# mtumalan/VisionTransformer

Measured on AMD Instinct MI355X. Metric: images/sec (512×512) ViT-B/16 seg, 1/2/4/8 MI355X + mask argmax match, higher is better.
Workload: dtype f32

## Files before the change

visiontransformer_amd/csrc/common.hpp:

```cpp
#pragma once
#include <hip/hip_runtime.h>
#include <stdint.h>

#include "../../include/vitseg.h"

namespace vitseg {

constexpr int WAVE = 64;

typedef float f32x4 __attribute__((ext_vector_type(4)));
typedef float f32x16 __attribute__((ext_vector_type(16)));
typedef short bf16x8 __attribute__((ext_vector_type(8)));
typedef short bf16x4 __attribute__((ext_vector_type(4)));

void set_error(const char* fmt, ...);
int hip_fail(hipError_t e, const char* what);

enum Opt {
    OPT_NO_F32P = 0,
    OPT_NO_P8,
    OPT_NO_H16P,
    OPT_NO_RAGGED_P8,
    OPT_NO_DROPMASK,
    OPT_DROPW_LIMIT_MB,
    OPT_UPSAMPLE_GLOBAL,
    OPT_BF16_TILES,
    OPT_F32P_NOINL,
    OPT_GN,
    OPT_NO_MASK2,
    OPT_NO_SMALL,
    OPT_SMALL_VARIANT,
    OPT_SMALL_MAX_ROWS,
    OPT_CONV_DMA,
    OPT_COUNT
};
long opt(int id);

#define VITSEG_CHECK_ARG(cond, code, ...) \
    do {                                  \
        if (!(cond)) {                    \
            ::vitseg::set_error(__VA_ARGS__); \
            return (code);                \
        }                                 \
    } while (0)

#define VITSEG_LAUNCH_CHECK(what)                               \
    do {                                                        \
        hipError_t e__ = hipGetLastError();                     \
        if (e__ != hipSuccess) return ::vitseg::hip_fail(e__, what); \
    } while (0)

inline size_t up256(size_t v) { return (v + 255) & ~(size_t)255; }

__device__ __forceinline__ int xcd_remap(int bid, int nwg) {
    const int q = nwg >> 3, r = nwg & 7, xcd = bid & 7, idx = bid >> 3;
    const int base = (xcd < r) ? xcd * (q + 1) : r * (q + 1) + (xcd - r) * q;
    return base + idx;
}

struct AttnTile {
    int rt, head, b;
};
__device__ __forceinline__ AttnTile attn_tile(int ntiles, int A) {
    const int t = xcd_remap(blockIdx.x, gridDim.x);
    const int bh = t / ntiles;
    AttnTile r;
    r.rt = t - bh * ntiles;
    r.b = bh / A;
    r.head = bh - r.b * A;
    return r;
}

__host__ __device__ __forceinline__ unsigned fmix32(unsigned h) {
    h ^= h >> 16;
    h *= 0x85ebca6bu;
    h ^= h >> 13;
    h *= 0xc2b2ae35u;
    h ^= h >> 16;
    return h;
}
__host__ __device__ __forceinline__ unsigned drop_key(unsigned seed, unsigned stream, unsigned major) {
    return fmix32(seed ^ (stream * 0x9E3779B1u) ^ (major * 0x85EBCA77u));
}
__host__ __device__ __forceinline__ unsigned mad24(unsigned a, unsigned k, unsigned c) {
#if defined(__HIP_DEVICE_COMPILE__)
    return __umul24(a, k) + c;
// ... 209 lines not shown
```

visiontransformer_amd/csrc/forward.hip:

```cpp
#include "kernels.hpp"
#include "profile.hpp"
#include "forward.hpp"

namespace vitseg {

using namespace plan;

long small_max_rows() {
    const long v = opt(OPT_SMALL_MAX_ROWS);
    return v > 0 ? v : SMALL_MAX_ROWS;
}

bool small_applies(const vitseg_config* cfg, int batch, int precision) {
    Shape s;
    if (precision == VITSEG_F32X3 || opt(OPT_NO_SMALL) || check_config(cfg, &s)) return false;
    const long rows = (long)batch * s.N;
    if (!(rows < small_max_rows() && s.D % 64 == 0 && s.I % 32 == 0 && s.I > s.D && s.S % 4 == 0)) return false;
    const long lim16 = opt(OPT_SMALL_MAX_ROWS) > 0 ? opt(OPT_SMALL_MAX_ROWS) : small_max_rows_16(s.N);
    if (precision != VITSEG_F32 && !(s.I % 64 == 0 && attn_small_infer(s.Np) && rows < lim16)) return false;
    if (precision != VITSEG_F32 && ((s.D / small_splits(s.D, s.D)) % 64 || (s.I / small_splits(s.D, s.I)) % 64)) return false;
    return true;
}

namespace {
// ... 22 lines not shown
    }
    if (int rc = launch_cls_rows(wt(f, VITSEG_T_CLS), f.pos, X, f.batch, s.Np, s.D, f.st)) return rc;
    if (f.drop_p > 0.f) return launch_dropout_rows(X, X, 0, Mp + f.batch, s.D, drop(f, 0, 0), f.st);
    return VITSEG_OK;
}

int head_conv_gemm(const Fwd& f) {
    const Shape& s = f.s;
    const int Mp = f.batch * s.Np, D = s.D;
    GemmArgs g{};
    g.A = f.hf; g.W = wg(f, VITSEG_T_HEAD0_W); g.bias = wt(f, VITSEG_T_HEAD0_B); g.C = f.F;
    g.M = Mp; g.N = MID; g.K = 9 * D; g.lda = 0; g.ldc = MID;
    g.g = s.g; g.Np = s.Np; g.D = D;
    g.zeros = f.zeros;
    if (f.h16) {
        hipError_t e = hipMemsetAsync((void*)f.zeros, 0, 256, f.st);
        if (e != hipSuccess) return hip_fail(e, "hipMemsetAsync(zero page)");
    }
    ProfScope ps(f.prof.conv3, 2.0 * g.M * g.N * g.K, f.st);
    if (f.conv_dma && !f.h16 && !f.x3 && D % 32 == 0 && opt(OPT_CONV_DMA) && (size_t)(Mp + 128) * D * 4 < 0x7fffffffull) {
        SGemm c{};
        c.A = (const float*)f.hf; c.W = wt(f, VITSEG_T_HEAD0_W); c.bias = wt(f, VITSEG_T_HEAD0_B); c.C = f.F;
        c.M = Mp; c.N = MID; c.K = D; c.lda = D; c.ldw = 9 * D; c.ldc = MID; c.splits = 1;
        c.g = s.g; c.Np = s.Np;
        return launch_gemm_f32s(c, SE_RELU, SA_CONV3_ALL, f.st);
    }
    return f.h16 ? launch_gemm_bf16(g, A_CONV3, EPI_RELU, f.st, f.h16 == 2) : launch_gemm_f32(g, A_CONV3, EPI_RELU, f.st, f.x3);
}

int head_1x1(const Fwd& f) {
    const Shape& s = f.s;
    const size_t Mp = (size_t)f.batch * s.Np;
    ProfScope ps(f.prof.head1x1, (double)Mp * MID * 4 + (double)f.batch * s.C * s.Np * 4, f.st);
    return launch_head1x1(f.F, wt(f, VITSEG_T_HEAD2_W), wt(f, VITSEG_T_HEAD2_B), f.Z, f.batch, s.Np, s.C, f.st);
}

int upsample(const Fwd& f) {
    const Shape& s = f.s;
    if (!f.logits && !f.mask) return VITSEG_OK;
    const double px = (double)f.batch * s.S * s.S;
    ProfScope ps(f.prof.upsample, (f.logits ? px * s.C * 4 : 0.0) + (f.mask ? px : 0.0) + (double)f.batch * s.C * s.Np * 4, f.st);
    return launch_upsample(f.Z, f.logits, f.mask, f.batch, s.C, s.g, s.S, f.st);
}

}

int walk_large(const Fwd& f) {
    const Shape& s = f.s;
    const int Mp = f.batch * s.Np, Mt = Mp + f.batch, D = s.D, I = s.I;
    hipStream_t st = f.st;
    int rc;
    if ((rc = embed_gemm(f, f.layer(0).xin, f.h16 ? 1 : f.x3))) return rc;
    const int thin_rows = f.thin_rows ? thin_cls_rows(Mp, f.batch) : 0;
    auto gemm = [&](const void* A, int w, int b, int l, const float* R, void* C, int N, int K, int epi, int kind,
                    DropArgs dr = DropArgs{}, void* aux = nullptr) {
        GemmArgs g{};
        g.A = A; g.W = wg(f, w, l); g.bias = wt(f, b, l); g.R = R; g.C = C; g.aux = aux; g.drop = dr;
        g.M = Mt; g.N = N; g.K = K; g.lda = K; g.ldc = N;
        if (f.whole_split || thin_rows) {
            g.thin_rows = thin_rows;
            g.thin_scratch = f.scratch;
            g.thin_capacity = f.scratch_floats;
        }
        ProfScope ps(kind, 2.0 * g.M * g.N * g.K, st);
        if (f.fc1_train && epi == EPI_GELU) return launch_gemm_bf16_train(g, EPI_GELU, st);
        return f.h16 ? launch_gemm_bf16(g, A_PLAIN, epi, st, f.h16 == 2) : launch_gemm_f32(g, A_PLAIN, epi, st, f.x3);
    };
    auto lnorm = [&](const float* X, int w, int b, int l, void* H, int rows) {
        ProfScope ps(f.prof.ln, (double)rows * D * (f.h16 ? 6 : 8), st);
        return launch_layernorm(X, wt(f, w, l), wt(f, b, l), H, rows, D, f.eps, f.h16, st);
    };
    const bool mlp1 = f.prof.mlp_one_scope;
    for (int l = 0; l < s.L; ++l) {
        const LayerIO io = f.layer(l);
        if ((rc = lnorm(io.xin, VITSEG_T_LN1_W, VITSEG_T_LN1_B, l, io.h1, Mt))) return rc;
        if ((rc = gemm(io.h1, VITSEG_T_WQKV, VITSEG_T_BQKV, l, nullptr, io.qkv, 3 * D, D, EPI_BIAS, f.prof.qkv))) return rc;
        {
            ProfScope ps(f.prof.attn, 4.0 * f.batch * s.A * (double)s.N * s.N * 64, st);
            const DropArgs dr = drop(f, l, 1);
            if (io.dropw && (rc = launch_attn_dropmask((unsigned*)io.dropw, f.batch, s.Np, s.A, dr, st))) return rc;
            rc = f.h16 ? launch_attention_bf16(io.qkv, io.ctx, io.lse, f.batch, s.Np, s.A, dr, st, f.h16 == 2, io.dropw)
                       : launch_attention_f32((const float*)io.qkv, (float*)io.ctx, io.lse, f.batch, s.Np, s.A, dr, st, f.x3 != 0);
            if (rc) return rc;
        }
        if ((rc = gemm(io.ctx, VITSEG_T_WO, VITSEG_T_BO, l, io.xin, io.xmid, D, D, EPI_RESADD, f.prof.oproj, drop(f, l, 2))))
            return rc;
        if ((rc = lnorm(io.xmid, VITSEG_T_LN2_W, VITSEG_T_LN2_B, l, io.h2, Mt))) return rc;
        ProfScope ps(mlp1 ? f.prof.fc1 : -1, 4.0 * Mt * D * I, st);
        if ((rc = gemm(io.h2, VITSEG_T_W1, VITSEG_T_B1, l, nullptr, io.uact, I, D, EPI_GELU, mlp1 ? -1 : f.prof.fc1, DropArgs{},
                       io.upre)))
            return rc;
        if ((rc = gemm(io.uact, VITSEG_T_W2, VITSEG_T_B2, l, io.xmid, io.xout, D, I, EPI_RESADD, mlp1 ? -1 : f.prof.fc2,
                       drop(f, l, 3))))
            return rc;
    }
    if ((rc = lnorm(f.layer(s.L - 1).xout, VITSEG_T_LNF_W, VITSEG_T_LNF_B, 0, f.hf, Mp))) return rc;
    if ((rc = head_conv_gemm(f)) || (rc = head_1x1(f))) return rc;
    return upsample(f);
}

int walk_small(const Fwd& f) {
    const Shape& s = f.s;
    const int Mp = f.batch * s.Np, Mt = Mp + f.batch, D = s.D;
    hipStream_t st = f.st;
    float* part = f.scratch;
    const size_t dstride = (size_t)Mt * D;
    int rc;
    auto linear = [&](const void* A, int K, int w, int b, int l, void* C, int N, int epi, void* aux, int kind) {
        SGemm g{};
        g.A = (const float*)A; g.W = (const float*)wg(f, w, l); g.bias = wt(f, b, l); g.C = (float*)C; g.aux = (float*)aux;
        g.h16 = f.h16;
        g.M = Mt; g.N = N; g.K = K; g.lda = K; g.ldw = K; g.ldc = N;
        g.splits = epi == SE_PARTIAL ? small_splits(N, K) : 1;
        g.split_stride = dstride;
        ProfScope ps(kind, 2.0 * g.M * g.N * g.K, st);
        return launch_gemm_f32s(g, epi, SA_PLAIN, st);
    };
    auto rows = [&](float* X, const float* Xres, int splits, const float* bias, DropArgs dr, int lnw, int lnb, int ln_layer,
                    void* H, int ln_rows, int h_fmt, bool embed) {
        SRows r{};
        r.h_fmt = h_fmt;
        r.X = X; r.Xres = Xres == X ? nullptr : Xres; r.partial = part; r.split_stride = dstride; r.splits = splits;
        r.bias = bias; r.drop = dr;
        r.pos = f.pos; r.cls = wt(f, VITSEG_T_CLS); r.lnw = wt(f, lnw, ln_layer); r.lnb = wt(f, lnb, ln_layer); r.H = (float*)H;
        r.rows = Mt; r.Mp = Mp; r.Np = s.Np; r.D = D; r.ln_rows = ln_rows; r.embed = embed ? 1 : 0;
        r.eps = f.eps;
        ProfScope ps(f.prof.ln, (double)Mt * D * 4 * (2 + splits) + (double)ln_rows * D * 4, st);
        return launch_resln(r, st);
    };
    const LayerIO io0 = f.layer(0);
    if ((s.P == 8 || s.P == 16 || s.P == 32) && s.Kp % 32 == 0) {
        SGemm g{};
        g.A = f.x; g.W = wt(f, VITSEG_T_PATCH_W); g.C = part;
        g.M = Mp; g.N = D; g.K = s.Kp; g.lda = 0; g.ldw = s.Kp; g.ldc = D;
        g.splits = small_splits(D, s.Kp); g.split_stride = dstride;
        g.g = s.g; g.Np = s.Np; g.S = s.S; g.P = s.P; g.Cin = s.Cin;
        {
            ProfScope ps(f.prof.patch, 2.0 * g.M * g.N * g.K, st);
            if ((rc = launch_gemm_f32s(g, SE_PARTIAL, SA_PATCH, st))) return rc;
        }
        if ((rc = rows(io0.xin, nullptr, g.splits, wt(f, VITSEG_T_PATCH_B), drop(f, 0, 0), VITSEG_T_LN1_W, VITSEG_T_LN1_B, 0,
                       io0.h1, Mt, f.h16, true)))
            return rc;
    } else {
        if ((rc = embed_gemm(f, io0.xin, 0))) return rc;
        ProfScope ps(f.prof.ln, (double)Mt * D * 8, st);
        if ((rc = launch_layernorm(io0.xin, wt(f, VITSEG_T_LN1_W), wt(f, VITSEG_T_LN1_B), io0.h1, Mt, D, f.eps, f.h16, st)))
            return rc;
    }
// ... 71 lines not shown
```

visiontransformer_amd/csrc/forward.hpp:

```cpp
#pragma once
#include <functional>

#include "plan.hpp"
#include "small.hpp"

namespace vitseg {

struct LayerIO {
    float* xin;
    void* h1;
    void* qkv;
    void* ctx;
    float* lse;
    float* xmid;
    void* h2;
    void* upre;
    void* uact;
    float* xout;
    const unsigned* dropw;
};

struct FwdProf {
    int patch, ln, qkv, attn, oproj, fc1, fc2, conv3, head1x1, upsample;
    bool mlp_one_scope;
};

struct Fwd {
    plan::Shape s;
    const plan::Layout* lay;
    const float* params;
    const void* params_lp;
    const float* pos;
    const float* x;
    int batch;
    float eps;
    hipStream_t st;
    int h16;
    int x3;
    std::function<LayerIO(int)> layer;
    void* hf;
    float* F;
    float* Z;
    const void* zeros;
    float* scratch;
    size_t scratch_floats;
    float* logits;
    uint8_t* mask;
    float drop_p;
    unsigned drop_seed;
    bool thin_rows;
    bool whole_split;
    bool fc1_train;
    bool (*attn_small)(int Np);
    bool head_one_chain;
    bool conv_dma;
    FwdProf prof;
};

int walk_large(const Fwd& f);
int walk_small(const Fwd& f);

enum SmallRole { SMALL_INFER, SMALL_TRAIN_FWD, SMALL_TRAIN_BWD };
size_t small_slab_floats(const plan::Shape& s, size_t Mt, size_t Mp, SmallRole role);

inline int thin_cls_rows(size_t Mp, int batch) { return Mp % 256 == 0 && batch <= THIN_MAX_ROWS ? batch : 0; }

}
```

visiontransformer_amd/csrc/gemm_dispatch.hip:

```cpp
#include "gemm_tiles.hpp"

namespace vitseg {
namespace {

int whole_split_shape(int M, int N, int K, int kstep) { return K % kstep == 0 ? whole_split(M, N, K, kstep) : 0; }

int thin_slices(int K, int kstep) {
    if (K < 256 || K % kstep != 0) return 0;
    const int sl = K / kstep / 4;
    return sl > THIN_MAX_SPLITS ? THIN_MAX_SPLITS : sl < 1 ? 1 : sl;
}

int whole_split_applies(const GemmArgs& a, int epi, int kstep) {
    const int sp = whole_split_shape(a.M, a.N, a.K, kstep);
    const bool ok = sp && a.thin_scratch && (size_t)sp * a.M * a.N <= a.thin_capacity && !a.drop.thresh &&
                    !a.aux && a.splitk <= 1 && a.ldc % 4 == 0 && (epi == EPI_BIAS || epi == EPI_GELU || epi == EPI_RESADD);
    return ok ? sp : 0;
}

int thin_split_applies(const GemmArgs& a, int epi, int kstep) {
    const bool h16 = kstep == 64;
    const int sl = thin_slices(a.K, kstep);
    const bool ok = sl && a.thin_scratch && a.thin_rows > 0 && a.thin_rows <= THIN_MAX_ROWS && a.M > a.thin_rows &&
                    (size_t)sl * a.thin_rows * a.N <= a.thin_capacity && (a.M - a.thin_rows) % BM == 0 &&
                    (h16 || (!a.drop.thresh && !a.aux)) && a.splitk <= 1 && a.ldc % 4 == 0 &&
                    (epi == EPI_BIAS || epi == EPI_GELU || epi == EPI_RESADD || (h16 && epi == EPI_DGELU));
    return ok ? sl : 0;
}

template <typename F>
int sliced(GemmArgs a, int splits, float* scratch, hipStream_t s, F launch) {
    float* out = (float*)a.C;
    if (splits > 1) {
        a.C = scratch;
        a.splitk = splits;
    }
    a.split_stride = (size_t)a.M * a.N;
    if (int rc = launch(a)) return rc;
    return splits > 1 ? launch_splitk_reduce(scratch, out, (size_t)a.M * a.N / 4, splits, s) : VITSEG_OK;
}

enum H16Kernel { HK_NONE, HK_TILE, HK_LARGE, HK_XL, HK_P8, HK_H16P };

struct H16Route {
    H16Kernel body;
    int body_rows;
    int tail_rows;
    int slices;
    int colsum_rows;
};

}

int launch_gemm_f32(const GemmArgs& a_in, int amode, int epi, hipStream_t s, int x3) {
    if (x3 != 1 && x3 != 2) x3 = 0;
    GemmArgs a = a_in;
    if (amode == A_PLAIN) {
        if (const int sp = whole_split_applies(a_in, epi, 32)) {
            a.thin_rows = a_in.M;
            return launch_thin_rows(GT_F32, x3, a, epi, sp, s);
        }
        if (const int sl = thin_split_applies(a_in, epi, 32)) {
            if (int rc = launch_thin_rows(GT_F32, x3, a_in, epi, sl, s)) return rc;
            a.M = a_in.M - a_in.thin_rows;
        }
    }
    a.thin_scratch = nullptr;
    VITSEG_CHECK_ARG(a.M > 0 && a.N > 0 && a.K > 0 && a.K % 4 == 0, VITSEG_EINVAL, "gemm_f32: bad M/N/K %d %d %d", a.M, a.N, a.K);
    VITSEG_CHECK_ARG(a.N % 4 == 0 && a.ldc % 4 == 0, VITSEG_ESHAPE, "gemm: N=%d and ldc=%d must be multiples of 4", a.N, a.ldc);
    if (amode == A_PLAIN) {
        VITSEG_CHECK_ARG(a.lda % 4 == 0, VITSEG_EINVAL, "gemm_f32: lda %% 4");
        if (!x3 && gemm_f32p_applies(a, epi)) return launch_gemm_f32p(a, epi, s);
    } else if (amode == A_PATCH && epi == EPI_POS) {
        VITSEG_CHECK_ARG(a.P % 4 == 0, VITSEG_ESHAPE, "patch size must be a multiple of 4");
    } else if (amode == A_CONV3 && epi == EPI_RELU) {
        VITSEG_CHECK_ARG(a.D % 4 == 0, VITSEG_ESHAPE, "hidden size must be a multiple of 4");
    }
    static const char* const who[3] = {"gemm_f32", "gemm_f32 (x3)", "gemm_f32 (x3, split W)"};
    return launch_gemm_tile(GT_F32, true, amode, epi, x3, a, s, who[x3]);
}

int launch_gemm_f32_bwd(const GemmArgs& a, int amode, int ta, int tb, int epi, hipStream_t s) {
    VITSEG_CHECK_ARG(a.M > 0 && a.N > 0 && a.K > 0, VITSEG_EINVAL, "gemm_bwd: bad M/N/K %d %d %d", a.M, a.N, a.K);
    VITSEG_CHECK_ARG(a.N % 4 == 0 && a.ldc % 4 == 0 && a.lda % 4 == 0 && a.ldw % 4 == 0, VITSEG_ESHAPE,
                     "gemm_bwd: leading dimensions must be multiples of 4");
    VITSEG_CHECK_ARG(ta || a.K % 4 == 0, VITSEG_ESHAPE, "gemm_bwd: K %% 4");
    VITSEG_CHECK_ARG(!ta || a.M % 4 == 0, VITSEG_ESHAPE, "gemm_bwd: M %% 4 for a T-form A");
    return launch_gemm_tile_bwd(amode, ta, tb, epi, a, s);
}

int launch_wgrad_f32(GemmArgs a, float* scratch, hipStream_t s) {
    const int splits = wgrad_splits(a.M, a.N, a.K, 32);
    VITSEG_CHECK_ARG(splits <= 1 || (a.ldc == a.N && scratch), VITSEG_EINVAL, "wgrad: split-K needs a dense output and scratch");
    return sliced(a, splits, scratch, s, [&](const GemmArgs& g) { return launch_gemm_f32_bwd(g, A_PLAIN, 1, 1, EPI_BIAS, s); });
}

static int route_h16(const GemmArgs& a_in, int amode, int epi, H16Route& r) {
    r = H16Route{HK_NONE, 0, 0, 0, 0};
    const bool want_cs = a_in.colsum_out && a_in.colsum_scratch && epi == EPI_DGELU;
    const auto persistent = [&](const GemmArgs& g) {
        r.body = gemm_h16p_applies(g, epi) ? HK_H16P : HK_P8;
        r.body_rows = g.M;
        r.colsum_rows = want_cs ? g.M : 0;
        return VITSEG_OK;
    };
    GemmArgs a = a_in;
    if (amode == A_PLAIN) {
        if (const int sp = whole_split_applies(a_in, epi, 64)) {
            r.tail_rows = a_in.M;
            r.slices = sp;
            return VITSEG_OK;
        }
        if (a_in.M % 256 != 0 && a_in.M % 256 <= 128 && gemm_p8_applies(a_in, epi) &&
            gemm_p8_rounds(a_in.M, a_in.N) == gemm_p8_rounds(a_in.M - a_in.M % 256, a_in.N) && !opt(OPT_NO_RAGGED_P8))
            return persistent(a_in);
        const int sl = (a_in.M - a_in.thin_rows) % LBM == 0 ? thin_split_applies(a_in, epi, 64) : 0;
        if (sl) {
            r.tail_rows = a_in.thin_rows;
            r.slices = sl;
// ... 20 lines not shown
        r.body = xl ? HK_XL : large ? HK_LARGE : HK_TILE;
        if (epi == EPI_BIAS || epi == EPI_GELU || epi == EPI_DGELU || epi == EPI_RESADD) return VITSEG_OK;
    } else if (amode == A_CONV3 && (epi == EPI_RELU || epi == EPI_BIAS)) {
        VITSEG_CHECK_ARG(a.D % 64 == 0 && a.zeros, VITSEG_ESHAPE, "%s must be a multiple of 64",
                         epi == EPI_RELU ? "hidden size" : "channel count");
        r.body = large ? HK_LARGE : HK_TILE;
        return VITSEG_OK;
    }
    set_error("gemm_bf16: unsupported amode/epilogue %d/%d", amode, epi);
    return VITSEG_EINVAL;
}

int launch_gemm_bf16(const GemmArgs& a_in, int amode, int epi, hipStream_t s, bool f16) {
    H16Route r;
    if (int rc = route_h16(a_in, amode, epi, r)) return rc;
    const GemmType type = f16 ? GT_F16 : GT_BF16;
    const bool out_f32 = epi == EPI_RESADD || amode == A_CONV3;
    GemmArgs a = a_in;
    if (r.slices) {
        a.thin_rows = r.tail_rows;
        if (int rc = launch_thin_rows(type, 0, a, epi, r.slices, s)) return rc;
    }
    a.M = r.body_rows;
    a.thin_scratch = nullptr;
    if (!r.colsum_rows) a.colsum_scratch = nullptr;
    int rc = VITSEG_OK;
    switch (r.body) {
        case HK_NONE: break;
        case HK_P8: rc = launch_gemm_p8(a, epi, s, f16); break;
        case HK_H16P: rc = launch_gemm_h16p(a, s, f16); break;
        case HK_XL: rc = launch_gemm_large(f16, amode, epi, 256, a, s, "gemm_bf16"); break;
        case HK_LARGE: rc = launch_gemm_large(f16, amode, epi, 128, a, s, "gemm_bf16"); break;
        case HK_TILE: rc = launch_gemm_tile(type, out_f32, amode, epi, 0, a, s, "gemm_bf16");
    }
    if (rc) return rc;
    if (r.tail_rows && !r.slices) {
        GemmArgs t = a;
        const auto row = [&](const void* p, size_t esz) { return (char*)p + (size_t)r.body_rows * a.ldc * esz; };
        t.M = r.tail_rows;
        t.row_base = a.row_base + r.body_rows;
        t.A = (const char*)a.A + (size_t)r.body_rows * a.lda * 2;
        if (a.aux) t.aux = row(a.aux, 2);
        if (a.R) t.R = (const float*)row(a.R, epi == EPI_RESADD ? 4 : 2);
        t.C = row(a.C, out_f32 ? 4 : 2);
        if ((rc = launch_gemm_tile(type, out_f32, A_PLAIN, epi, 0, t, s, "gemm_bf16"))) return rc;
    }
    if (!a_in.colsum_out) return VITSEG_OK;
    VITSEG_CHECK_ARG(a_in.colsum_scratch && !f16, VITSEG_EINVAL, "gemm: column sums need bf16 + scratch");
    if (r.colsum_rows > 0)
        return launch_colsum_finish_fused((const bf16_t*)a_in.C + (size_t)r.colsum_rows * a_in.ldc, a_in.M - r.colsum_rows,
                                          2 * ((r.colsum_rows + 255) / 256), a_in.colsum_out, a_in.colsum_scratch, a_in.N,
                                          a_in.ldc, s);
    return launch_colsum(a_in.C, 1, a_in.colsum_out, a_in.colsum_scratch, a_in.M, a_in.N, a_in.ldc, s);
}

int launch_wgrad_bf16_tt(GemmArgs a, float* scratch, hipStream_t s) {
    VITSEG_CHECK_ARG(a.M % 8 == 0 && a.N % 8 == 0 && a.lda % 8 == 0 && a.ldw % 8 == 0 && a.ldc == a.N && a.zeros,
                     VITSEG_ESHAPE, "wgrad_bf16_tt: M, N and the leading dimensions must be multiples of 8");
    if (wgrad_p8_applies(a)) return launch_wgrad_p8(a, scratch, s);
    const int splits = wgrad_bf16_splits(a.M, a.N, a.K, false);
    VITSEG_CHECK_ARG(splits <= 1 || scratch, VITSEG_EINVAL, "wgrad_bf16_tt: split-K needs scratch");
    return sliced(a, splits, scratch, s, [&](const GemmArgs& g) { return launch_gemm_tt(g, s); });
}

int launch_gemm_bf16_train(const GemmArgs& a, int epi, hipStream_t s) {
    VITSEG_CHECK_ARG(a.M > 0 && a.N > 0 && a.K > 0 && a.K % 64 == 0, VITSEG_ESHAPE, "gemm_bf16_train: K=%d %% 64", a.K);
    VITSEG_CHECK_ARG(a.N % 4 == 0 && a.ldc % 4 == 0 && a.lda % 8 == 0, VITSEG_ESHAPE, "gemm_bf16_train: alignment");
    if (epi == EPI_BIAS || epi == EPI_GELU || epi == EPI_DGELU) return launch_gemm_bf16(a, A_PLAIN, epi, s, false);
    set_error("gemm_bf16_train: unsupported epilogue %d", epi);
    return VITSEG_EINVAL;
}

int gemm_slices(int path, int M, int N, int K) {
    if (M <= 0 || N <= 0 || K <= 0) return 0;
    GemmArgs g{};
    g.M = M; g.N = N; g.K = K; g.lda = M; g.ldw = N; g.ldc = N;
    const bool tt_ok = M % 8 == 0 && N % 8 == 0;
    switch (path) {
        case VITSEG_SLICES_WHOLE_F32: return whole_split_shape(M, N, K, 32);
        case VITSEG_SLICES_WHOLE_H16: return whole_split_shape(M, N, K, 64);
        case VITSEG_SLICES_THIN_F32: return thin_slices(K, 32);
        case VITSEG_SLICES_THIN_H16: return thin_slices(K, 64);
        case VITSEG_SLICES_WGRAD_F32: return wgrad_splits(M, N, K, 32);
        case VITSEG_SLICES_WGRAD_BF16_TT: return tt_ok && !wgrad_p8_applies(g) ? wgrad_bf16_splits(M, N, K, false) : 0;
        case VITSEG_SLICES_WGRAD_BF16_P8: return tt_ok && wgrad_p8_applies(g) ? wgrad_bf16_splits(M, N, K, true) : 0;
    }
    return 0;
}

}
```

visiontransformer_amd/csrc/kernels.hpp:

```cpp
#pragma once
#include "common.hpp"

namespace vitseg {

enum AMode {
    A_PLAIN = 0,
    A_PATCH = 1,
    A_CONV3 = 2
};
enum Epi {
    EPI_BIAS = 0,
    EPI_GELU = 1,
    EPI_RESADD = 2,
    EPI_RELU = 3,
    EPI_POS = 4,
    EPI_DGELU = 5
};

struct GemmArgs {
    const void* A;
    const void* W;
    const float* bias;
    const float* R;
    void* C;
    int M, N, K;
    int lda, ldc;
    int ldw;
    void* aux;
    float* colsum_out;
    float* colsum_scratch;
    int S, P, g, Np, Cin, D;
    const void* zeros;
    int splitk;
    size_t split_stride;
    float* thin_scratch;
    size_t thin_capacity;
    int thin_rows;
    int gn;
    DropArgs drop;
    int row_base;
};

constexpr int THIN_MAX_SPLITS = 16, THIN_MAX_ROWS = 64;
inline size_t thin_scratch_floats(int max_n) { return (size_t)THIN_MAX_SPLITS * THIN_MAX_ROWS * max_n; }
inline int whole_split(int M, int N, int K, int kstep) {
    const int tiles = ((M + 127) / 128) * ((N + 127) / 128);
    if (tiles > 128 || K < 512) return 0;
    int s = K / kstep / 4;
    if (s > 8) s = 8;
    return s >= 2 ? s : 0;
}
int launch_gemm_f32(const GemmArgs& a, int amode, int epi, hipStream_t s, int x3 = 0);
int launch_gemm_f32_bwd(const GemmArgs& a, int amode, int ta, int tb, int epi, hipStream_t s);
size_t wgrad_scratch_floats(int M, int N, int K);
int launch_wgrad_f32(GemmArgs a, float* scratch, hipStream_t s);
int launch_wgrad_bf16_tt(GemmArgs a, float* scratch, hipStream_t s);
int launch_gemm_bf16_train(const GemmArgs& a, int epi, hipStream_t s);
size_t wgrad_bf16_scratch_floats(int M, int N, int K);
int wgrad_bf16_splits(int M, int N, int K, bool p8);
int gemm_slices(int path, int M, int N, int K);
int launch_gemm_bf16(const GemmArgs& a, int amode, int epi, hipStream_t s, bool f16 = false);
int gemm_p8_rounds(int M, int N);
int device_num_cus();
bool gemm_p8_applies(const GemmArgs& a, int epi);
int launch_gemm_p8(const GemmArgs& a, int epi, hipStream_t s, bool f16);
bool gemm_h16p_applies(const GemmArgs& a, int epi);
int launch_gemm_h16p(const GemmArgs& a, hipStream_t s, bool f16);
bool gemm_f32p_applies(const GemmArgs& a, int epi);
int launch_gemm_f32p(const GemmArgs& a, int epi, hipStream_t s);
bool wgrad_p8_applies(const GemmArgs& a);
int wgrad_p8_splits(int M, int N, int K);
int launch_wgrad_p8(GemmArgs a, float* scratch, hipStream_t s);
int launch_splitk_reduce(const float* partial, float* out, size_t n4, int splits, hipStream_t s);

int launch_layernorm(const float* x, const float* w, const float* b, void* y, int rows, int D, float eps,
                     int out_fmt, hipStream_t s);

int launch_attention_f32(const float* qkv, float* ctx, float* lse, int B, int Np, int A, DropArgs dr, hipStream_t s,
                         bool x3 = false);
int launch_attention_x3_main(const float* qkv, float* ctx, int B, int Np, int A, hipStream_t s);
int launch_attention_bwd_f32(const float* qkv, const float* ctx, const float* dctx, const float* lse, float* dvec,
                             float* dqkv, int B, int Np, int A, DropArgs dr, hipStream_t s);
int launch_attention_bf16(const void* qkv, void* ctx, float* lse, int B, int Np, int A, DropArgs dr, hipStream_t s,
                          bool f16 = false, const unsigned* maskw = nullptr);
size_t attention_bwd_bf16_scratch_floats(int B, int Np, int A);
int launch_attention_bwd_bf16(const void* qkv, const void* ctx, const void* dctx, const float* lse, float* dvec,
                              void* dqkv, int B, int Np, int A, DropArgs dr, hipStream_t s,
                              const unsigned* maskw = nullptr, float* dbias = nullptr);
int launch_attn_dropmask(unsigned* W, int B, int Np, int A, DropArgs dr, hipStream_t s);

int launch_head1x1(const float* F, const float* W2, const float* b2, float* Z, int B, int Np, int C, hipStream_t s);
int launch_upsample(const float* Z, float* logits, uint8_t* mask, int B, int C, int g, int S, hipStream_t s);
int window_count(int extent, int S, int stride);
int launch_window_gather(const void* src, int src_is_u8, int n, int H, int W, int S, const int* oy, int ny, const int* ox,
                         int nx, int first, int count, float* out, hipStream_t s);
int launch_window_blend(const float* lowres, const int* oy, int ny, const int* ox, int nx, const float* w, int n, int C, int g,
                        int S, int H, int W, float* logits, uint8_t* mask, hipStream_t s);

size_t ce_partial_count(int B, int S);
int launch_ce_loss(const float* Z, const void* target, int target_is_u8, float* G, double* partial, float* loss, int B,
                   int C, int g, int S, hipStream_t s, float gscale = 1.0f);
size_t ce_opts_scratch_bytes(int B, int S);
int check_ce_options(const vitseg_ce_options& o, int B, int C, int S);
int launch_ce_loss_opts(const float* Z, const void* target, int target_is_u8, float* G, double* partial, float* loss, int B,
                        int C, int g, int S, const vitseg_ce_options& opts, hipStream_t s, float gscale = 1.0f);
// ... 83 lines not shown
```

visiontransformer_amd/csrc/vitseg_api.hip:

```cpp
#include <ctype.h>
#include <stdarg.h>
#include <stdio.h>
#include <stdlib.h>
#include <strings.h>

#include <atomic>

#include <vector>

#include "kernels.hpp"
#include "profile.hpp"
#include "forward.hpp"

namespace vitseg {

static thread_local char g_err[512] = "";

void set_error(const char* fmt, ...) {
    va_list ap;
    va_start(ap, fmt);
    vsnprintf(g_err, sizeof(g_err), fmt, ap);
    va_end(ap);
}

int hip_fail(hipError_t e, const char* what) {
    set_error("%s: %s", what, hipGetErrorString(e));
    return VITSEG_EHIP;
}

static const char* const g_opt_names[OPT_COUNT] = {"no_f32p", "no_p8", "no_h16p", "no_ragged_p8", "no_dropmask",
                                                   "dropw_limit_mb", "upsample_global", "bf16_tiles", "f32p_noinl", "gn", "no_mask2", "no_small",
                                                   "small_variant", "small_max_rows", "conv_dma"};
static std::atomic<long> g_opts[OPT_COUNT];
static int opt_index(const char* name) {
    if (!name) return -1;
    for (int i = 0; i < OPT_COUNT; ++i)
        if (!strcasecmp(name, g_opt_names[i])) return i;
    return -1;
}
static long opt_parse(int id, const char* text) {
    if (id == OPT_BF16_TILES && (text[0] == 's' || text[0] == 'l' || text[0] == 'x')) return text[0] == 's' ? 1 : text[0] == 'l' ? 2 : 3;
    char* end = nullptr;
    const long v = strtol(text, &end, 10);
    if (end != text) return v;
    return (id == OPT_DROPW_LIMIT_MB || id == OPT_GN || id == OPT_SMALL_VARIANT || id == OPT_SMALL_MAX_ROWS || id == OPT_BF16_TILES) ? 0 : 1;
}
static const bool g_opts_loaded = [] {
    for (int i = 0; i < OPT_COUNT; ++i) {
        char env[64] = "VITSEG_";
        for (size_t k = 0; g_opt_names[i][k] && k + 8 < sizeof(env); ++k) {
            env[7 + k] = (char)toupper((unsigned char)g_opt_names[i][k]);
            env[8 + k] = 0;
        }
        const char* e = getenv(env);
        g_opts[i].store(e ? opt_parse(i, e) : (i == OPT_DROPW_LIMIT_MB ? -1 : 0), std::memory_order_relaxed);
    }
    return true;
}();
long opt(int id) { return g_opts[id].load(std::memory_order_relaxed); }

namespace {

using namespace plan;

struct Plan {
    size_t zero, x, h, qkv, u, f, z, thin, pos, total;
    size_t thin_floats;
    size_t Mt, Mp;
};

Plan make_plan(const Shape& s, int B, int precision, bool pos_interp = false) {
    Plan p{};
    p.Mp = (size_t)B * s.Np;
    p.Mt = p.Mp + B;
    const size_t act = (precision == VITSEG_F32 || precision == VITSEG_F32X3) ? 4 : 2;
    size_t off = 0;
    auto take = [&](size_t bytes) {
        const size_t o = off;
        off += up(bytes, 256);
        return o;
    };
    p.zero = take(256);
    p.x = take(p.Mt * s.D * 4);
    p.h = take(p.Mt * s.D * 4);
    const bool small_rows = precision != VITSEG_F32X3 && (long)p.Mt < small_max_rows();
    p.qkv = take(p.Mt * 3 * s.D * (small_rows ? 4 : act));
    p.u = take(p.Mt * (size_t)s.I * act);
    p.f = take(p.Mp * MID * 4);
    p.z = take((size_t)B * s.C * s.Np * 4);
    const int widest = 3 * s.D > s.I ? 3 * s.D : s.I;
    p.thin_floats = thin_scratch_floats(widest);
    const int shapes[4][2] = {{3 * s.D, s.D}, {s.D, s.D}, {s.I, s.D}, {s.D, s.I}};
    for (auto& nk : shapes) {
        const size_t need = (size_t)whole_split((int)p.Mt, nk[0], nk[1], 32) * p.Mt * nk[0];
        if (need > p.thin_floats) p.thin_floats = need;
    }
    if (small_rows) {
        const size_t need = small_slab_floats(s, p.Mt, p.Mp, SMALL_INFER);
        if (need > p.thin_floats) p.thin_floats = need;
    }
    p.thin = take(p.thin_floats * 4);
    if (pos_interp) p.pos = take((size_t)s.N * s.D * 4);
    p.total = off;
    return p;
}

}

Profiler& profiler() {
    static Profiler p;
    return p;
}

}

using namespace vitseg;

extern "C" {

int vitseg_version(void) { return VITSEG_VERSION; }
const char* vitseg_last_error(void) { return g_err; }

int vitseg_set_option(const char* name, long long value) {
    const int id = opt_index(name);
    VITSEG_CHECK_ARG(id >= 0, VITSEG_EINVAL, "vitseg_set_option: unknown option '%s'", name ? name : "(null)");
    g_opts[id].store((long)value, std::memory_order_relaxed);
    return VITSEG_OK;
}
int vitseg_get_option(const char* name, long long* value) {
    const int id = opt_index(name);
    VITSEG_CHECK_ARG(id >= 0 && value, VITSEG_EINVAL, "vitseg_get_option: unknown option '%s'", name ? name : "(null)");
    *value = opt(id);
    return VITSEG_OK;
}

int vitseg_param_count(const vitseg_config* cfg, size_t* n_floats) {
    Shape s;
    if (int rc = check_config(cfg, &s)) return rc;
    VITSEG_CHECK_ARG(n_floats, VITSEG_EINVAL, "n_floats is null");
    *n_floats = make_layout(s).total;
    return VITSEG_OK;
}

int vitseg_param_offset(const vitseg_config* cfg, int tensor, int layer, size_t* offset_floats, size_t* numel) {
    Shape s;
    if (int rc = check_config(cfg, &s)) return rc;
    VITSEG_CHECK_ARG(tensor >= 0 && tensor < VITSEG_T_COUNT, VITSEG_EINVAL, "tensor id %d", tensor);
    VITSEG_CHECK_ARG(!per_layer(tensor) || (layer >= 0 && layer < s.L), VITSEG_EINVAL, "layer %d out of range", layer);
    const Layout l = make_layout(s);
    if (offset_floats) *offset_floats = tensor_offset(l, tensor, layer);
    if (numel) *numel = tensor_numel(s, tensor);
    return VITSEG_OK;
}

int vitseg_cast_params_bf16(const float* params, void* params_bf16, size_t n_floats, void* stream) {
    VITSEG_CHECK_ARG(params && params_bf16, VITSEG_EINVAL, "null arena");
    return launch_cast_bf16(params, params_bf16, n_floats, (hipStream_t)stream);
}

int vitseg_cast_params_split(const float* params, void* params_split, size_t n_floats, void* stream) {
    VITSEG_CHECK_ARG(params && params_split, VITSEG_EINVAL, "null arena");
    return launch_cast_split(params, params_split, n_floats, (hipStream_t)stream);
}

int vitseg_cast_params_f16(const float* params, void* params_f16, size_t n_floats, void* stream) {
    VITSEG_CHECK_ARG(params && params_f16, VITSEG_EINVAL, "null arena");
// ... 40 lines not shown
        case VITSEG_BUF_LOWRES: o = p.z; n = (size_t)batch * s.C * s.Np * 4; break;
        default: set_error("buffer id %d", buffer); return VITSEG_EINVAL;
    }
    if (offset_bytes) *offset_bytes = o;
    if (bytes) *bytes = n;
    return VITSEG_OK;
}

int vitseg_forward(const vitseg_config* cfg, const float* params, const void* params_bf16, const float* x, int batch,
                   int precision, float* logits, uint8_t* mask, void* workspace, size_t workspace_bytes,
                   void* stream_) {
    return vitseg_forward_at(cfg, cfg ? cfg->image_size : 0, params, params_bf16, x, batch, precision, logits, mask, workspace,
                             workspace_bytes, stream_);
}

static int forward_walk(const vitseg_config* cfg, int image_size_in, const float* params, const void* params_bf16, const float* x,
                        int batch, int precision, float* logits, uint8_t* mask, float* lowres, void* workspace,
                        size_t workspace_bytes, void* stream_) {
    Shape s, s0;
    vitseg_config cin;
    if (int rc = derive_input(cfg, image_size_in, &cin, &s, &s0)) return rc;
    VITSEG_CHECK_ARG(params && x && workspace && batch >= 1, VITSEG_EINVAL, "null pointer or batch < 1");
    VITSEG_CHECK_ARG(lowres || logits || mask, VITSEG_EINVAL, "both outputs are null");
    VITSEG_CHECK_ARG(precision >= VITSEG_F32 && precision <= VITSEG_F32X3, VITSEG_EINVAL, "precision %d", precision);
    if (int rc = check_precision(s, precision)) return rc;
    VITSEG_CHECK_ARG(precision == VITSEG_F32 || precision == VITSEG_F32X3 || params_bf16, VITSEG_EINVAL,
                     "16-bit forward needs the 16-bit arena");
    VITSEG_CHECK_ARG(((uintptr_t)params | (uintptr_t)x | (uintptr_t)workspace | (uintptr_t)logits) % 16 == 0,
                     VITSEG_EINVAL, "pointers must be 16-byte aligned");
    const Plan p = make_plan(s, batch, precision, s.g != s0.g);
    VITSEG_CHECK_ARG(workspace_bytes >= p.total, VITSEG_EWORKSPACE, "workspace %zu < required %zu", workspace_bytes,
                     p.total);
    hipStream_t st = (hipStream_t)stream_;
    const Layout lay = make_layout(s0);
    char* ws = (char*)workspace;
    const float* pos = params + tensor_offset(lay, VITSEG_T_POS, 0);
    if (s.g != s0.g) {
        float* table = (float*)(ws + p.pos);
        if (int rc = launch_pos_interp(pos, table, s0.g, s.g, s.D, st)) return rc;
        pos = table;
    }
    float* X = (float*)(ws + p.x);
    void* H = ws + p.h;
    const LayerIO io{X, H, ws + p.qkv, H, nullptr, X, H, nullptr, ws + p.u, X, nullptr};
    Fwd f{};
    f.s = s; f.lay = &lay; f.params = params; f.params_lp = params_bf16; f.pos = pos; f.x = x; f.batch = batch;
    f.eps = cfg->layer_norm_eps; f.st = st;
    f.h16 = precision == VITSEG_BF16 ? 1 : precision == VITSEG_F16 ? 2 : 0;
    f.x3 = precision == VITSEG_F32X3 ? (params_bf16 ? 2 : 1) : 0;
    f.layer = [&](int) { return io; };
    f.hf = H; f.F = (float*)(ws + p.f); f.Z = lowres ? lowres : (float*)(ws + p.z); f.zeros = ws + p.zero;
    f.scratch = (float*)(ws + p.thin); f.scratch_floats = p.thin_floats;
    f.logits = logits; f.mask = mask;
    f.thin_rows = true; f.whole_split = true; f.attn_small = attn_small_infer; f.conv_dma = true;
    f.prof = FwdProf{VITSEG_K_GEMM_PATCH, VITSEG_K_LAYERNORM, VITSEG_K_GEMM_BIAS, VITSEG_K_ATTENTION, VITSEG_K_GEMM_RESADD,
                     VITSEG_K_GEMM_GELU, VITSEG_K_GEMM_RESADD, VITSEG_K_GEMM_CONV3, VITSEG_K_HEAD1X1, VITSEG_K_UPSAMPLE, false};
    return small_applies(&cin, batch, precision) ? walk_small(f) : walk_large(f);
}

int vitseg_forward_at(const vitseg_config* cfg, int image_size_in, const float* params, const void* params_bf16, const float* x,
                      int batch, int precision, float* logits, uint8_t* mask, void* workspace, size_t workspace_bytes,
                      void* stream_) {
    return forward_walk(cfg, image_size_in, params, params_bf16, x, batch, precision, logits, mask, nullptr, workspace,
                        workspace_bytes, stream_);
}

int vitseg_forward_lowres(const vitseg_config* cfg, int image_size_in, const float* params, const void* params_bf16,
                          const float* x, int batch, int precision, float* lowres, void* workspace, size_t workspace_bytes,
                          void* stream_) {
    VITSEG_CHECK_ARG(lowres, VITSEG_EINVAL, "forward_lowres: the output is null");
    return forward_walk(cfg, image_size_in, params, params_bf16, x, batch, precision, nullptr, nullptr, lowres, workspace,
                        workspace_bytes, stream_);
}

size_t vitseg_ce_scratch_bytes(int batch, int S) { return ce_partial_count(batch, S) * sizeof(double); }

int vitseg_ce_loss(const float* lowres, const void* target, int target_is_u8, float* grad_logits, void* scratch,
                   float* loss, int batch, int C, int g, int S, void* stream) {
    VITSEG_CHECK_ARG(batch >= 1 && C >= 1 && g >= 1 && S >= g, VITSEG_EINVAL, "ce_loss: bad shape");
    return launch_ce_loss(lowres, target, target_is_u8, grad_logits, (double*)scratch, loss, batch, C, g, S,
                          (hipStream_t)stream);
}

size_t vitseg_ce_options_scratch_bytes(int batch, int S) {
    return batch >= 1 && S >= 1 ? ce_opts_scratch_bytes(batch, S) : 0;
}

int vitseg_ce_loss_opts(const float* lowres, const void* target, int target_is_u8, float* grad_logits, void* scratch,
                        float* loss, int batch, int C, int g, int S, const vitseg_ce_options* opts, float loss_scale,
                        void* stream) {
    VITSEG_CHECK_ARG(batch >= 1 && C >= 1 && g >= 1 && S >= g, VITSEG_EINVAL, "ce_loss: bad shape");
    if (!opts)
        return launch_ce_loss(lowres, target, target_is_u8, grad_logits, (double*)scratch, loss, batch, C, g, S,
                              (hipStream_t)stream, loss_scale);
    return launch_ce_loss_opts(lowres, target, target_is_u8, grad_logits, (double*)scratch, loss, batch, C, g, S, *opts,
                               (hipStream_t)stream, loss_scale);
}

size_t vitseg_dice_options_scratch_bytes(int batch, int C, int S) {
    return batch >= 1 && C >= 1 && S >= 1 ? dice_scratch_bytes(batch, C, S) : 0;
}

int vitseg_ce_dice_loss(const float* lowres, const void* target, int target_is_u8, float* grad_logits, void* scratch,
                        float* terms, int batch, int C, int g, int S, const vitseg_ce_options* ce,
                        const vitseg_dice_options* dice, float loss_scale, void* stream) {
    VITSEG_CHECK_ARG(batch >= 1 && C >= 1 && g >= 1 && S >= g, VITSEG_EINVAL, "ce_dice_loss: bad shape");
    VITSEG_CHECK_ARG(dice, VITSEG_EINVAL, "ce_dice_loss: the dice options are null");
// ... 393 lines not shown
```

Before: 614.3.

## Run CLS-token thin-row GEMM and layernorm work on a side stream

In the large f32 forward path, the thin CLS-row portion of each split GEMM and the CLS rows of each layernorm are moved onto a per-device side stream. Events order that stream against the main stream, so this small work overlaps with the main patch-row GEMMs and attention instead of serializing with them. The option is on by default. It is skipped when the stream is being captured and for bf16 and x3 precision. It adds event record and wait overhead per layer, plus a shared per-device side stream and event ring, which could contend across concurrent callers.

```diff
diff --git a/visiontransformer_amd/csrc/common.hpp b/visiontransformer_amd/csrc/common.hpp
--- a/visiontransformer_amd/csrc/common.hpp
+++ b/visiontransformer_amd/csrc/common.hpp
@@ -32,6 +32,7 @@
     OPT_SMALL_VARIANT,
     OPT_SMALL_MAX_ROWS,
     OPT_CONV_DMA,
+    OPT_CLS_OVERLAP,
     OPT_COUNT
 };
 long opt(int id);
diff --git a/visiontransformer_amd/csrc/forward.hip b/visiontransformer_amd/csrc/forward.hip
--- a/visiontransformer_amd/csrc/forward.hip
+++ b/visiontransformer_amd/csrc/forward.hip
@@ -98,8 +98,42 @@
     int rc;
     if ((rc = embed_gemm(f, f.layer(0).xin, f.h16 ? 1 : f.x3))) return rc;
     const int thin_rows = f.thin_rows ? thin_cls_rows(Mp, f.batch) : 0;
-    auto gemm = [&](const void* A, int w, int b, int l, const float* R, void* C, int N, int K, int epi, int kind,
-                    DropArgs dr = DropArgs{}, void* aux = nullptr) {
+    auto cuts = [&](int N, int K, int epi) {
+        GemmArgs g{};
+        g.M = Mt; g.N = N; g.K = K; g.lda = K; g.ldc = N;
+        g.thin_rows = thin_rows; g.thin_scratch = f.scratch; g.thin_capacity = f.scratch_floats;
+        return gemm_splits_thin(g, epi);
+    };
+    SideLane* lane = nullptr;
+    if (f.cls_side && thin_rows && !f.h16 && !f.x3 && opt(OPT_CLS_OVERLAP) && cuts(3 * D, D, EPI_BIAS) && cuts(D, D, EPI_RESADD) &&
+        cuts(I, D, EPI_GELU) && cuts(D, I, EPI_RESADD)) {
+        hipStreamCaptureStatus cap = hipStreamCaptureStatusNone;
+        if (hipStreamIsCapturing(st, &cap) != hipSuccess) {
+            (void)hipGetLastError();
+            cap = hipStreamCaptureStatusActive;
+        }
+        if (cap == hipStreamCaptureStatusNone && !(lane = side_lane())) return VITSEG_EHIP;
+    }
+    hipStream_t sd = lane ? lane->st : nullptr;
+    bool side_busy = false;
+    auto order = [&](hipStream_t from, hipStream_t to) -> int {
+        hipEvent_t ev = lane->event();
+        hipError_t e = hipEventRecord(ev, from);
+        if (e == hipSuccess) e = hipStreamWaitEvent(to, ev, 0);
+        return e == hipSuccess ? VITSEG_OK : hip_fail(e, "walk_large: stream order");
+    };
+    auto to_side = [&]() -> int { return lane ? order(st, sd) : VITSEG_OK; };
+    auto to_main = [&]() -> int {
+        if (!side_busy) return VITSEG_OK;
+        side_busy = false;
+        return order(sd, st);
+    };
+    struct Join {
+        decltype(to_main)& f;
+        ~Join() { (void)f(); }
+    } join{to_main};
+    auto gemm = [&](const void* A, int w, int b, int l, const float* R, void* C, int N, int K, int epi, int kind, bool gate,
+                    DropArgs dr = DropArgs{}, void* aux = nullptr) -> int {
         GemmArgs g{};
         g.A = A; g.W = wg(f, w, l); g.bias = wt(f, b, l); g.R = R; g.C = C; g.aux = aux; g.drop = dr;
         g.M = Mt; g.N = N; g.K = K; g.lda = K; g.ldc = N;
@@ -108,19 +142,38 @@
             g.thin_scratch = f.scratch;
             g.thin_capacity = f.scratch_floats;
         }
-        ProfScope ps(kind, 2.0 * g.M * g.N * g.K, st);
-        if (f.fc1_train && epi == EPI_GELU) return launch_gemm_bf16_train(g, EPI_GELU, st);
-        return f.h16 ? launch_gemm_bf16(g, A_PLAIN, epi, st, f.h16 == 2) : launch_gemm_f32(g, A_PLAIN, epi, st, f.x3);
-    };
-    auto lnorm = [&](const float* X, int w, int b, int l, void* H, int rows) {
-        ProfScope ps(f.prof.ln, (double)rows * D * (f.h16 ? 6 : 8), st);
-        return launch_layernorm(X, wt(f, w, l), wt(f, b, l), H, rows, D, f.eps, f.h16, st);
-    };
+        auto run = [&](hipStream_t on, GemmPart part) -> int {
+            if (f.fc1_train && epi == EPI_GELU) return launch_gemm_bf16_train(g, EPI_GELU, on);
+            return f.h16 ? launch_gemm_bf16(g, A_PLAIN, epi, on, f.h16 == 2) : launch_gemm_f32(g, A_PLAIN, epi, on, f.x3, part);
+        };
+        {
+            ProfScope ps(kind, 2.0 * g.M * g.N * g.K, st);
+            if (int r = run(st, lane ? GEMM_BODY : GEMM_WHOLE)) return r;
+        }
+        if (!lane) return VITSEG_OK;
+        if (gate)
+            if (int r = to_side()) return r;
+        side_busy = true;
+        return run(sd, GEMM_THIN);
+    };
+    auto lnorm = [&](const float* X, int w, int b, int l, void* H, int rows) -> int {
+        const int main_rows = lane && rows == Mt ? Mp : rows;
+        {
+            ProfScope ps(f.prof.ln, (double)main_rows * D * (f.h16 ? 6 : 8), st);
+            if (int r = launch_layernorm(X, wt(f, w, l), wt(f, b, l), H, main_rows, D, f.eps, f.h16, st)) return r;
+        }
+        if (main_rows == rows) return VITSEG_OK;
+        side_busy = true;
+        return launch_layernorm(X + (size_t)Mp * D, wt(f, w, l), wt(f, b, l), (char*)H + (size_t)Mp * D * (f.h16 ? 2 : 4), f.batch, D,
+                                f.eps, f.h16, sd);
+    };
+    if ((rc = to_side())) return rc;
     const bool mlp1 = f.prof.mlp_one_scope;
     for (int l = 0; l < s.L; ++l) {
         const LayerIO io = f.layer(l);
         if ((rc = lnorm(io.xin, VITSEG_T_LN1_W, VITSEG_T_LN1_B, l, io.h1, Mt))) return rc;
-        if ((rc = gemm(io.h1, VITSEG_T_WQKV, VITSEG_T_BQKV, l, nullptr, io.qkv, 3 * D, D, EPI_BIAS, f.prof.qkv))) return rc;
+        if ((rc = gemm(io.h1, VITSEG_T_WQKV, VITSEG_T_BQKV, l, nullptr, io.qkv, 3 * D, D, EPI_BIAS, f.prof.qkv, false))) return rc;
+        if ((rc = to_main())) return rc;
         {
             ProfScope ps(f.prof.attn, 4.0 * f.batch * s.A * (double)s.N * s.N * 64, st);
             const DropArgs dr = drop(f, l, 1);
@@ -129,18 +182,20 @@
                        : launch_attention_f32((const float*)io.qkv, (float*)io.ctx, io.lse, f.batch, s.Np, s.A, dr, st, f.x3 != 0);
             if (rc) return rc;
         }
-        if ((rc = gemm(io.ctx, VITSEG_T_WO, VITSEG_T_BO, l, io.xin, io.xmid, D, D, EPI_RESADD, f.prof.oproj, drop(f, l, 2))))
+        if ((rc = gemm(io.ctx, VITSEG_T_WO, VITSEG_T_BO, l, io.xin, io.xmid, D, D, EPI_RESADD, f.prof.oproj, true,
+                       drop(f, l, 2))))
             return rc;
         if ((rc = lnorm(io.xmid, VITSEG_T_LN2_W, VITSEG_T_LN2_B, l, io.h2, Mt))) return rc;
         ProfScope ps(mlp1 ? f.prof.fc1 : -1, 4.0 * Mt * D * I, st);
-        if ((rc = gemm(io.h2, VITSEG_T_W1, VITSEG_T_B1, l, nullptr, io.uact, I, D, EPI_GELU, mlp1 ? -1 : f.prof.fc1, DropArgs{},
-                       io.upre)))
+        if ((rc = gemm(io.h2, VITSEG_T_W1, VITSEG_T_B1, l, nullptr, io.uact, I, D, EPI_GELU, mlp1 ? -1 : f.prof.fc1, false,
+                       DropArgs{}, io.upre)))
             return rc;
         if ((rc = gemm(io.uact, VITSEG_T_W2, VITSEG_T_B2, l, io.xmid, io.xout, D, I, EPI_RESADD, mlp1 ? -1 : f.prof.fc2,
-                       drop(f, l, 3))))
+                       true, drop(f, l, 3))))
             return rc;
     }
     if ((rc = lnorm(f.layer(s.L - 1).xout, VITSEG_T_LNF_W, VITSEG_T_LNF_B, 0, f.hf, Mp))) return rc;
+    if ((rc = to_main())) return rc;
     if ((rc = head_conv_gemm(f)) || (rc = head_1x1(f))) return rc;
     return upsample(f);
 }
diff --git a/visiontransformer_amd/csrc/forward.hpp b/visiontransformer_amd/csrc/forward.hpp
--- a/visiontransformer_amd/csrc/forward.hpp
+++ b/visiontransformer_amd/csrc/forward.hpp
@@ -1,4 +1,5 @@
 #pragma once
+#include <atomic>
 #include <functional>
 
 #include "plan.hpp"
@@ -54,8 +55,17 @@
     bool (*attn_small)(int Np);
     bool head_one_chain;
     bool conv_dma;
+    bool cls_side;
     FwdProf prof;
 };
+
+struct SideLane {
+    hipStream_t st = nullptr;
+    hipEvent_t ev[64] = {};
+    std::atomic<unsigned> next{0};
+    hipEvent_t event() { return ev[next.fetch_add(1, std::memory_order_relaxed) % 64]; }
+};
+SideLane* side_lane();
 
 int walk_large(const Fwd& f);
 int walk_small(const Fwd& f);
diff --git a/visiontransformer_amd/csrc/gemm_dispatch.hip b/visiontransformer_amd/csrc/gemm_dispatch.hip
--- a/visiontransformer_amd/csrc/gemm_dispatch.hip
+++ b/visiontransformer_amd/csrc/gemm_dispatch.hip
@@ -52,19 +52,26 @@
 
 }
 
-int launch_gemm_f32(const GemmArgs& a_in, int amode, int epi, hipStream_t s, int x3) {
+int launch_gemm_f32(const GemmArgs& a_in, int amode, int epi, hipStream_t s, int x3, GemmPart part) {
     if (x3 != 1 && x3 != 2) x3 = 0;
     GemmArgs a = a_in;
-    if (amode == A_PLAIN) {
-        if (const int sp = whole_split_applies(a_in, epi, 32)) {
+    bool split = false;
+    if (amode == A_PLAIN) {
+        const int sp = whole_split_applies(a_in, epi, 32);
+        if (sp && part == GEMM_WHOLE) {
             a.thin_rows = a_in.M;
             return launch_thin_rows(GT_F32, x3, a, epi, sp, s);
         }
-        if (const int sl = thin_split_applies(a_in, epi, 32)) {
-            if (int rc = launch_thin_rows(GT_F32, x3, a_in, epi, sl, s)) return rc;
+        const int sl = sp ? 0 : thin_split_applies(a_in, epi, 32);
+        if (sl) {
+            if (part != GEMM_BODY)
+                if (int rc = launch_thin_rows(GT_F32, x3, a_in, epi, sl, s)) return rc;
             a.M = a_in.M - a_in.thin_rows;
-        }
-    }
+            split = true;
+        }
+    }
+    VITSEG_CHECK_ARG(part == GEMM_WHOLE || split, VITSEG_EINVAL, "gemm_f32: this GEMM has no side launch to take apart (gemm_splits_thin)");
+    if (part == GEMM_THIN) return VITSEG_OK;
     a.thin_scratch = nullptr;
     VITSEG_CHECK_ARG(a.M > 0 && a.N > 0 && a.K > 0 && a.K % 4 == 0, VITSEG_EINVAL, "gemm_f32: bad M/N/K %d %d %d", a.M, a.N, a.K);
     VITSEG_CHECK_ARG(a.N % 4 == 0 && a.ldc % 4 == 0, VITSEG_ESHAPE, "gemm: N=%d and ldc=%d must be multiples of 4", a.N, a.ldc);
@@ -191,6 +198,10 @@
                                           2 * ((r.colsum_rows + 255) / 256), a_in.colsum_out, a_in.colsum_scratch, a_in.N,
                                           a_in.ldc, s);
     return launch_colsum(a_in.C, 1, a_in.colsum_out, a_in.colsum_scratch, a_in.M, a_in.N, a_in.ldc, s);
+}
+
+bool gemm_splits_thin(const GemmArgs& a, int epi) {
+    return !whole_split_applies(a, epi, 32) && thin_split_applies(a, epi, 32) > 0;
 }
 
 int launch_wgrad_bf16_tt(GemmArgs a, float* scratch, hipStream_t s) {
diff --git a/visiontransformer_amd/csrc/kernels.hpp b/visiontransformer_amd/csrc/kernels.hpp
--- a/visiontransformer_amd/csrc/kernels.hpp
+++ b/visiontransformer_amd/csrc/kernels.hpp
@@ -50,7 +50,9 @@
     if (s > 8) s = 8;
     return s >= 2 ? s : 0;
 }
-int launch_gemm_f32(const GemmArgs& a, int amode, int epi, hipStream_t s, int x3 = 0);
+enum GemmPart { GEMM_WHOLE = 0, GEMM_BODY, GEMM_THIN };
+bool gemm_splits_thin(const GemmArgs& a, int epi);
+int launch_gemm_f32(const GemmArgs& a, int amode, int epi, hipStream_t s, int x3 = 0, GemmPart part = GEMM_WHOLE);
 int launch_gemm_f32_bwd(const GemmArgs& a, int amode, int ta, int tb, int epi, hipStream_t s);
 size_t wgrad_scratch_floats(int M, int N, int K);
 int launch_wgrad_f32(GemmArgs a, float* scratch, hipStream_t s);
diff --git a/visiontransformer_amd/csrc/vitseg_api.hip b/visiontransformer_amd/csrc/vitseg_api.hip
--- a/visiontransformer_amd/csrc/vitseg_api.hip
+++ b/visiontransformer_amd/csrc/vitseg_api.hip
@@ -5,7 +5,7 @@
 #include <strings.h>
 
 #include <atomic>
-
+#include <mutex>
 #include <vector>
 
 #include "kernels.hpp"
@@ -30,7 +30,7 @@
 
 static const char* const g_opt_names[OPT_COUNT] = {"no_f32p", "no_p8", "no_h16p", "no_ragged_p8", "no_dropmask",
                                                    "dropw_limit_mb", "upsample_global", "bf16_tiles", "f32p_noinl", "gn", "no_mask2", "no_small",
-                                                   "small_variant", "small_max_rows", "conv_dma"};
+                                                   "small_variant", "small_max_rows", "conv_dma", "cls_overlap"};
 static std::atomic<long> g_opts[OPT_COUNT];
 static int opt_index(const char* name) {
     if (!name) return -1;
@@ -53,7 +53,7 @@
             env[8 + k] = 0;
         }
         const char* e = getenv(env);
-        g_opts[i].store(e ? opt_parse(i, e) : (i == OPT_DROPW_LIMIT_MB ? -1 : 0), std::memory_order_relaxed);
+        g_opts[i].store(e ? opt_parse(i, e) : (i == OPT_DROPW_LIMIT_MB ? -1 : i == OPT_CLS_OVERLAP ? 1 : 0), std::memory_order_relaxed);
     }
     return true;
 }();
@@ -112,6 +112,32 @@
     return p;
 }
 
+SideLane* side_lane() {
+    static std::mutex mu;
+    static std::vector<SideLane*> lanes;
+    int dev = 0;
+    hipError_t e = hipGetDevice(&dev);
+    if (e != hipSuccess || dev < 0) {
+        hip_fail(e, "hipGetDevice");
+        return nullptr;
+    }
+    std::lock_guard<std::mutex> lock(mu);
+    if ((size_t)dev >= lanes.size()) lanes.resize(dev + 1, nullptr);
+    if (lanes[dev]) return lanes[dev];
+    SideLane* l = new SideLane;
+    e = hipStreamCreateWithFlags(&l->st, hipStreamNonBlocking);
+    for (int i = 0; e == hipSuccess && i < 64; ++i) e = hipEventCreateWithFlags(&l->ev[i], hipEventDisableTiming);
+    if (e != hipSuccess) {
+        hip_fail(e, "side stream");
+        for (hipEvent_t ev : l->ev)
+            if (ev) (void)hipEventDestroy(ev);
+        if (l->st) (void)hipStreamDestroy(l->st);
+        delete l;
+        return nullptr;
+    }
+    return lanes[dev] = l;
+}
+
 }
 
 using namespace vitseg;
@@ -258,7 +284,7 @@
     f.hf = H; f.F = (float*)(ws + p.f); f.Z = lowres ? lowres : (float*)(ws + p.z); f.zeros = ws + p.zero;
     f.scratch = (float*)(ws + p.thin); f.scratch_floats = p.thin_floats;
     f.logits = logits; f.mask = mask;
-    f.thin_rows = true; f.whole_split = true; f.attn_small = attn_small_infer; f.conv_dma = true;
+    f.thin_rows = true; f.whole_split = true; f.attn_small = attn_small_infer; f.conv_dma = true; f.cls_side = true;
     f.prof = FwdProf{VITSEG_K_GEMM_PATCH, VITSEG_K_LAYERNORM, VITSEG_K_GEMM_BIAS, VITSEG_K_ATTENTION, VITSEG_K_GEMM_RESADD,
                      VITSEG_K_GEMM_GELU, VITSEG_K_GEMM_RESADD, VITSEG_K_GEMM_CONV3, VITSEG_K_HEAD1X1, VITSEG_K_UPSAMPLE, false};
     return small_applies(&cin, batch, precision) ? walk_small(f) : walk_large(f);
```

New measurement: 617.0, median of 6. About the same (+0.4%).
